# toandaominh1997/EfficientDet.Pytorch

Measured on NVIDIA H100. Metric: EfficientDet-D0 512x512 images/sec (fwd+bwd), higher is better.
Workload: dtype f32

## Files before the change

### efficientdet.pytorch_b200/csrc/conv_planes.cu

```cuda
#include "tc_ptx.cuh"

#include <stdlib.h>

namespace effdet {

constexpr int kPlMaxLevels = 8;
constexpr int kPlThreads = 384;
constexpr int kPlProducerRegs = 40, kPlConsumerRegs = 232;
constexpr int kPlA = 128 * 128;
template <int BN>
struct PlCfg {
    static constexpr int kStages = BN == 128 ? 3 : 4;
    static constexpr int kB = BN * 128;
    static constexpr int kStage = 2 * kPlA + 2 * kB;
    static constexpr int kSmem = kStages * kStage + kRowsBytes + 1024 + 256 + 2 * BN * 4;
};
constexpr int kPlBarRows = 2, kPlBarTurn = 4;

struct PlLevel {
    int B, H, W;
    WgGeom g;
    int tile_begin;
    int nboxes;
    float* y;
    long long y_bstride;
    __nv_bfloat16* y_planes;
    const __nv_bfloat16* mask_planes;
    const float* residual;
    long long r_bstride;
};
struct PlArgs {
    PlLevel lv[kPlMaxLevels];
    int nlevels, total_tiles, ntn;
    int Cin, Cout, ksize, act, kblocks, opitch;
    const float* bias;
    float* colsum;
};
struct PlMaps {
    CUtensorMap x[kPlMaxLevels];
};

template <int BN, int NP>
__global__ void __launch_bounds__(kPlThreads, 1)
conv_planes_kernel(const __grid_constant__ PlMaps maps, const __grid_constant__ CUtensorMap wmap, const __grid_constant__ PlArgs P) {
    constexpr int kPlBN = BN, kPlStages = PlCfg<BN>::kStages, kPlB = PlCfg<BN>::kB, kPlStage = PlCfg<BN>::kStage;
    extern __shared__ uint8_t smem_raw[];
    uint8_t* smem = smem_raw + ((1024u - (smem_u32(smem_raw) & 1023u)) & 1023u);
    float* rows_buf = reinterpret_cast<float*>(smem + kPlStages * kPlStage);
    uint64_t* full_bar = reinterpret_cast<uint64_t*>(smem + kPlStages * kPlStage + kRowsBytes);
    uint64_t* empty_bar = full_bar + kPlStages;
    float* chan_buf = reinterpret_cast<float*>(smem + kPlStages * kPlStage + kRowsBytes + 256);

    const int warp = threadIdx.x >> 5, lane = threadIdx.x & 31;
    const int taps = P.ksize * P.ksize, pad = P.ksize / 2;
    const int KT = taps * P.kblocks;
    if (threadIdx.x == 0) {
        for (int s = 0; s < kPlStages; ++s) {
            mbar_init(&full_bar[s], 1);
            mbar_init(&empty_bar[s], 4);
        }
        fence_barrier_init();
        tma_prefetch_desc(&wmap);
    }
    __syncthreads();

    auto decode = [&](int unit, int& l, int& box0, int& n0) {
        const int mt = unit / P.ntn;
        n0 = (unit - mt * P.ntn) * kPlBN;
        l = 0;
        while (l + 1 < P.nlevels && mt >= P.lv[l + 1].tile_begin) ++l;
        box0 = (mt - P.lv[l].tile_begin) * (128 / P.lv[l].g.kstage);
    };

    if (warp >= 8) {
        setmaxnreg_dec<kPlProducerRegs>();
        if (warp == 8 && lane == 0) {
            uint32_t it = 0;
            for (int unit = blockIdx.x; unit < P.total_tiles; unit += gridDim.x) {
                int l, box0, n0;
                decode(unit, l, box0, n0);
                const PlLevel& L = P.lv[l];
                const int ks = L.g.kstage, nbox = 128 / ks;
                const int nvalid = min(nbox, L.nboxes - box0);
                for (int kt = 0; kt < KT; ++kt, ++it) {
                    const int s = it % kPlStages;
                    const uint32_t ph = (it / kPlStages) & 1;
                    const int tap = kt / P.kblocks, kb = kt - tap * P.kblocks;
                    const int dy = tap / P.ksize - pad, dx = tap % P.ksize - pad;
                    mbar_wait(&empty_bar[s], ph ^ 1);
                    uint8_t* a_hi = smem + s * kPlStage;
                    uint8_t* b_hi = a_hi + 2 * kPlA;
                    mbar_arrive_expect_tx(&full_bar[s], (uint32_t)((NP == 3 ? 2 : 1) * (nvalid * ks * 128 + kPlB)));
                    for (int q = 0; q < nvalid; ++q) {
                        int ch = box0 + q;
                        const int bx = ch % L.g.nbx;
                        ch /= L.g.nbx;
                        const int by = ch % L.g.nby;
                        const int bb = ch / L.g.nby;
                        const int x0 = bx * L.g.Wb + dx, y0 = by * L.g.Hb + dy, b0 = bb * L.g.Bb;
                        tma_load_5d(a_hi + q * ks * 128, &maps.x[l], &full_bar[s], kb * 64, x0, y0, b0, 0);
                        if (NP == 3) tma_load_5d(a_hi + kPlA + q * ks * 128, &maps.x[l], &full_bar[s], kb * 64, x0, y0, b0, 1);
                    }
                    tma_load_3d(b_hi, &wmap, &full_bar[s], kt * 64, n0, 0);
                    if (NP == 3) tma_load_3d(b_hi + kPlB, &wmap, &full_bar[s], kt * 64, n0, 1);
                }
            }
        }
    } else {
        setmaxnreg_inc<kPlConsumerRegs>();
        constexpr int NB = kPlBN / 64;
        const int g = warp >> 2;
        const int half = (warp >> 1) & 1;
        const int etid = threadIdx.x & 127;
        float* rows = rows_buf + g * 32 * kRowsPitch;
        float* chan = chan_buf + g * kPlBN;
        const int nunits = (P.total_tiles - (int)blockIdx.x + (int)gridDim.x - 1) / (int)gridDim.x;
        int chan_n0 = -1;
        for (int k = g; k < nunits; k += 2) {
            int l, box0, n0;
            decode(blockIdx.x + k * gridDim.x, l, box0, n0);
            const PlLevel& L = P.lv[l];
            if (k > 0) named_bar_sync(kPlBarTurn + g, 256);
            float d[2][NB][32];
            uint32_t it = (uint32_t)k * KT;
            for (int kt = 0; kt < KT; ++kt, ++it) {
                const int s = it % kPlStages;
                const uint32_t ph = (it / kPlStages) & 1;
                mbar_wait(&full_bar[s], ph);
                const uint32_t sa = smem_u32(smem + s * kPlStage);
                const uint32_t sb = sa + 2 * kPlA;
                wgmma_fence();
#pragma unroll
                for (int k16 = 0; k16 < 4; ++k16) {
#pragma unroll
                    for (int m = 0; m < 2; ++m)
                        wg_mma<NB, 0, NP>(d[m], sa + m * 64 * 128 + k16 * 32, sa + kPlA + m * 64 * 128 + k16 * 32, sb + k16 * 32,
                                          sb + kPlB + k16 * 32, 16, 1024, (kt | k16) != 0);
                }
                wgmma_commit();
                wgmma_wait<1>();
                if (kt > 0 && lane == 0) mbar_arrive(&empty_bar[(it - 1) % kPlStages]);
            }
            if (k + 1 < nunits) named_bar_arrive(kPlBarTurn + (g ^ 1), 256);
            wgmma_wait<0>();
            if (lane == 0) mbar_arrive(&empty_bar[(it - 1) % kPlStages]);
            if (n0 != chan_n0) {
                named_bar_sync(kPlBarRows + g, 128);
                for (int i = etid; i < kPlBN; i += 128) chan[i] = (n0 + i < P.Cout && P.bias) ? __ldg(P.bias + n0 + i) : 0.f;
                named_bar_sync(kPlBarRows + g, 128);
                chan_n0 = n0;
            }
            const long long plane = (long long)L.B * L.H * L.W * P.opitch;
            const int ncols = min(kPlBN, P.Cout - n0);
            const int nchunks = (ncols + 31) >> 5;
#pragma unroll
            for (int m = 0; m < 2; ++m) {
                const int r = m * 64 + (warp & 1) * 32 + lane;
                const int ks = L.g.kstage;
                const int q = r / ks, i = r - q * ks;
                int ch = box0 + q;
                bool row_ok = ch < L.nboxes;
                const int bx = ch % L.g.nbx;
                ch /= L.g.nbx;
                const int by = ch % L.g.nby;
                const int bb = ch / L.g.nby;
                const int wh = L.g.Wb * L.g.Hb;
                const int bi = i / wh, rem = i - bi * wh;
                const int yy = rem / L.g.Wb, xx = rem - yy * L.g.Wb;
                const int b = bb * L.g.Bb + bi, y = by * L.g.Hb + yy, x = bx * L.g.Wb + xx;
                row_ok = row_ok && b < L.B;
// ... 248 lines not shown
```

### efficientdet.pytorch_b200/csrc/conv_tc.cu

```cuda
#include "tc_ptx.cuh"

namespace effdet {

constexpr int kTcThreads = 288;
constexpr int kTcProducers = 256;
constexpr int kTileM = 128;
constexpr int kTileK = 64;
constexpr int kWgMaxChunksPerSplit = 64;

template <int BN, int STAGES>
struct FwdSmem {
    static constexpr int kA = kTileM * 128;
    static constexpr int kB = BN * 128;
    static constexpr int kStage = 2 * kA + 2 * kB;
    static constexpr int kChan = BN * 4;
    static constexpr int kBytes = STAGES * kStage + 1024  + 256  + kChan;
};

struct ConvMultiArgs {
    ConvLevel lv[kMaxLevels];
    int tile_begin[kMaxLevels + 1];
    int nlevels;
};

// ... 126 lines not shown
        for (int jb = 0; jb < NB; ++jb) {
            float acc[32];
            wg_rows<2>(d[jb], rows_buf, g, acc);
            const int cc = 2 * jb + half;
            if (cc >= nchunks || !row_ok) continue;
#pragma unroll
            for (int q = 0; q < 8; ++q) {
                const int nl = cc * 32 + q * 4;
                const int n = n0 + nl;
                if (n >= p.Cout) break;
                float4 v = make_float4(acc[q * 4], acc[q * 4 + 1], acc[q * 4 + 2], acc[q * 4 + 3]);
                v = f4add(v, *reinterpret_cast<const float4*>(chan + nl));
                if (p.act == EFFDET_ACT_RELU) {
                    v = make_float4(fmaxf(v.x, 0.f), fmaxf(v.y, 0.f), fmaxf(v.z, 0.f), fmaxf(v.w, 0.f));
                } else if (p.act == EFFDET_ACT_SIGMOID) {
                    v = make_float4(sigmoidf_(v.x), sigmoidf_(v.y), sigmoidf_(v.z), sigmoidf_(v.w));
                } else if (p.act == EFFDET_ACT_SWISH) {
                    v = make_float4(swishf_(v.x), swishf_(v.y), swishf_(v.z), swishf_(v.w));
                }
                if (p.residual) v = f4add(v, ldg4(p.residual + rbase + n));
                if (p.mask_src) {
                    const float4 mv = ldg4(p.mask_src + mbase + n);
                    v = make_float4(mv.x > 0.f ? v.x : 0.f, mv.y > 0.f ? v.y : 0.f, mv.z > 0.f ? v.z : 0.f, mv.w > 0.f ? v.w : 0.f);
                }
                st4(p.y + ybase + n, v);
            }
        }
    } else if (warp == 8) {
        if (lane == 0) {
            for (int kt = 0; kt < KT; ++kt) {
                const int s = kt % STAGES;
                const uint32_t ph = (kt / STAGES) & 1;
                mbar_wait(&empty_bar[s], ph ^ 1);
                uint8_t* b_hi = smem + s * S::kStage + 2 * S::kA;
                mbar_arrive_expect_tx(&full_bar[s], (NP == 3 ? 2 : 1) * S::kB);
                tma_load_3d(b_hi, &wmap, &full_bar[s], kt * kTileK, n0, 0);
                if (NP == 3) tma_load_3d(b_hi + S::kB, &wmap, &full_bar[s], kt * kTileK, n0, 1);
            }
        }
    }
}

template <int BC, int STAGES>
struct WgSmem {
    static constexpr int kA = kTileK * 128 * (kTileM / 64);
    static constexpr int kB = kTileK * 128 * (BC / 64);
    static constexpr int kStage = 2 * kA + 2 * kB;
    static constexpr int kBytes = STAGES * kStage + 1024 + 256;
};

template <int NGROUPS, int NP>
__device__ __forceinline__ void wg_produce(const float* __restrict__ src, const long long bstride, const int C, const int c0,
                                           const int H, const int W, const int HW, const int M, const int mbase, const int dy,
                                           const int dx, uint8_t* hi_plane, uint8_t* lo_plane, const int t) {
    constexpr int ITEMS = 64 * NGROUPS * 8 / kTcProducers;
    const int j = t & 7;
#pragma unroll 4
    for (int it = 0; it < ITEMS; ++it) {
        const int idx = it * kTcProducers + t;
        const int rg = idx >> 3;
        const int g = rg % NGROUPS, r = rg / NGROUPS;
        const int m = mbase + r;
        const int c = c0 + g * 64 + j * 8;
        float4 v0 = f4zero(), v1 = f4zero();
        if (m < M && c < C) {
            const int b = m / HW;
            const int pix = m - b * HW;
            const int oy = pix / W;
            const int iy = oy + dy, ix = pix - oy * W + dx;
            if (iy >= 0 && iy < H && ix >= 0 && ix < W) {
                const float* q = src + (long long)b * bstride + ((long long)iy * W + ix) * C + c;
                v0 = ldg4(q);
                if (c + 4 < C) v1 = ldg4(q + 4);
            }
        }
        if constexpr (NP == 3) {
            uint4 hi, lo;
            split8(v0, v1, hi, lo);
            const int off = g * (kTileK * 128) + r * 128 + ((j ^ (r & 7)) << 4);
            *reinterpret_cast<uint4*>(hi_plane + off) = hi;
            *reinterpret_cast<uint4*>(lo_plane + off) = lo;
        } else {
            const int off = g * (kTileK * 128) + r * 128 + ((j ^ (r & 7)) << 4);
            *reinterpret_cast<uint4*>(hi_plane + off) = hi8(v0, v1);
        }
    }
}

template <int NB>
__device__ __forceinline__ void wg_atomic_dw(const float (&d)[NB][32], float* dw, const int n0, const int c0, const int Cout,
                                             const int Cin, const int kk, const int tap) {
    const int w = (threadIdx.x >> 5) & 3, lane = threadIdx.x & 31;
#pragma unroll
    for (int jb = 0; jb < NB; ++jb)
#pragma unroll
        for (int i = 0; i < 32; ++i) {
            const int n = n0 + 16 * w + (lane >> 2) + 8 * ((i >> 1) & 1);
            const int c = c0 + jb * 64 + 8 * (i >> 2) + 2 * (lane & 3) + (i & 1);
            if (n < Cout && c < Cin) atomicAdd(dw + ((long long)n * Cin + c) * kk + tap, d[jb][i]);
        }
}

template <int BC, int STAGES, int NP>
__global__ void __launch_bounds__(kTcProducers, 1)
wgrad_tc_kernel(const __grid_constant__ WgradPrefix pa, const int M, const int HW, const int chunks_per_split, const int ctiles) {
    using S = WgSmem<BC, STAGES>;
    const effdet_wgrad_args& p = pa.get();
    extern __shared__ uint8_t smem_raw[];
    uint8_t* smem = smem_raw + ((1024u - (smem_u32(smem_raw) & 1023u)) & 1023u);

    const int warp = threadIdx.x >> 5;
    const int ct = blockIdx.x % ctiles, nt = blockIdx.x / ctiles;
    const int c0 = ct * BC, n0 = nt * kTileM;
    const int tap = blockIdx.y;
    const int pad = p.ksize / 2;
    const int dy = tap / p.ksize - pad, dx = tap % p.ksize - pad;
    const int nchunks = (M + kTileK - 1) / kTileK;
    const int ch_begin = blockIdx.z * chunks_per_split;
    const int ch_end = min(nchunks, ch_begin + chunks_per_split);
    const int KT = ch_end - ch_begin;
    constexpr int NB = BC / 64;
    constexpr uint32_t GROUP = kTileK * 128;
    const int t = threadIdx.x, g = warp >> 2;
    float d[NB][32];
    for (int kt = 0; kt < KT; ++kt) {
        const int s = kt % STAGES;
        wgmma_wait<STAGES - 1>();
        named_bar_sync(1, kTcProducers);
        uint8_t* a_hi = smem + s * S::kStage;
        uint8_t* b_hi = a_hi + 2 * S::kA;
        const int mbase = (ch_begin + kt) * kTileK;
        wg_produce<kTileM / 64, NP>(p.dy, p.dy_bstride, p.Cout, n0, p.H, p.W, HW, M, mbase, 0, 0, a_hi, a_hi + S::kA, t);
        wg_produce<BC / 64, NP>(p.x, p.x_bstride, p.Cin, c0, p.H, p.W, HW, M, mbase, dy, dx, b_hi, b_hi + S::kB, t);
        fence_proxy_async();
        named_bar_sync(1, kTcProducers);
        const uint32_t sa = smem_u32(a_hi) + g * GROUP, sb = smem_u32(b_hi);
        wg_mma_mn_steps<kTileK / 16, NP>(d, sa, sa + S::kA, sb, sb + S::kB, GROUP, kt != 0);
        wgmma_commit();
    }
    wgmma_wait<0>();
    wg_atomic_dw<NB>(d, p.dw, n0 + 64 * g, c0, p.Cout, p.Cin, p.ksize * p.ksize, tap);
}

struct WgMaps {
    CUtensorMap dy[kWgMaxLevels];
    CUtensorMap x[kWgMaxLevels];
};
struct WgMultiArgs {
    WgGeom g[kWgMaxLevels];
    int chunk_begin[kWgMaxLevels + 1];
    int nlevels;
    float* dw;
    int Cin, Cout, ksize;
};

template <int BC, int STAGES, int NP>
__global__ void __launch_bounds__(kTcThreads, 1)
wgrad_tc2_multi_kernel(const __grid_constant__ WgMaps maps, const __grid_constant__ WgMultiArgs a, const int chunks_per_split,
                       const int ctiles) {
    using S = WgSmem<BC, STAGES>;
    extern __shared__ uint8_t smem_raw[];
    uint8_t* smem = smem_raw + ((1024u - (smem_u32(smem_raw) & 1023u)) & 1023u);
    uint64_t* full_bar = reinterpret_cast<uint64_t*>(smem + STAGES * S::kStage);
    uint64_t* empty_bar = full_bar + STAGES;

    const int warp = threadIdx.x >> 5, lane = threadIdx.x & 31;
    const int ct = blockIdx.x % ctiles, nt = blockIdx.x / ctiles;
    const int c0 = ct * BC, n0 = nt * kTileM;
    const int tap = blockIdx.y;
    const int pad = a.ksize / 2;
    const int dy = tap / a.ksize - pad, dx = tap % a.ksize - pad;
    const int nchunks = a.chunk_begin[a.nlevels];
    const int ch_begin = blockIdx.z * chunks_per_split;
    const int ch_end = min(nchunks, ch_begin + chunks_per_split);
    const int KT = ch_end - ch_begin;

    if (threadIdx.x == 0) {
        for (int s = 0; s < STAGES; ++s) {
            mbar_init(&full_bar[s], 1);
            mbar_init(&empty_bar[s], 8);
        }
        fence_barrier_init();
    }
    __syncthreads();
    constexpr int GROUP = kTileK * 128;

    if (warp == 8) {
        if (lane == 0) {
            int l = 0;
            for (int kt = 0; kt < KT; ++kt) {
                const int s = kt % STAGES;
                const uint32_t ph = (kt / STAGES) & 1;
                const int chg = ch_begin + kt;
                while (l + 1 < a.nlevels && chg >= a.chunk_begin[l + 1]) ++l;
                const WgGeom& g = a.g[l];
                int ch = chg - a.chunk_begin[l];
                const int bx = ch % g.nbx;
                ch /= g.nbx;
                const int by = ch % g.nby;
                const int bb = ch / g.nby;
                const int x0 = bx * g.Wb, y0 = by * g.Hb, b0 = bb * g.Bb;
                const uint32_t bytes = (uint32_t)((NP == 3 ? 2 : 1) * (kTileM / 64 + BC / 64) * g.kstage * 128);
                mbar_wait(&empty_bar[s], ph ^ 1);
                mbar_arrive_expect_tx(&full_bar[s], bytes);
                uint8_t* a_hi = smem + s * S::kStage;
                uint8_t* b_hi = a_hi + 2 * S::kA;
#pragma unroll
                for (int pl = 0; pl < (NP == 3 ? 2 : 1); ++pl) {
#pragma unroll
                    for (int q = 0; q < kTileM / 64; ++q)
                        tma_load_5d(a_hi + pl * S::kA + q * GROUP, &maps.dy[l], &full_bar[s], n0 + q * 64, x0, y0, b0, pl);
#pragma unroll
                    for (int q = 0; q < BC / 64; ++q)
                        tma_load_5d(b_hi + pl * S::kB + q * GROUP, &maps.x[l], &full_bar[s], c0 + q * 64, x0 + dx, y0 + dy, b0, pl);
                }
            }
        }
    } else {
        constexpr int NB = BC / 64;
        const int wg = warp >> 2;
        float d[NB][32];
        for (int kt = 0, l = 0; kt < KT; ++l) {
            const int end = min(KT, a.chunk_begin[l + 1] - ch_begin);
            with_count<1, 2, 3, 4>(a.g[l].kstage / 16, [&](auto ksteps) {
                for (; kt < end; ++kt) {
                    const int s = kt % STAGES;
                    const uint32_t ph = (kt / STAGES) & 1;
                    mbar_wait(&full_bar[s], ph);
                    const uint32_t sa = smem_u32(smem + s * S::kStage) + wg * GROUP;
                    const uint32_t sb = smem_u32(smem + s * S::kStage) + 2 * S::kA;
                    wg_mma_mn_steps<ksteps, NP>(d, sa, sa + S::kA, sb, sb + S::kB, GROUP, kt != 0);
                    wgmma_commit();
                    wgmma_wait<1>();
                    if (kt > 0 && lane == 0) mbar_arrive(&empty_bar[(kt - 1) % STAGES]);
                }
            });
        }
        wgmma_wait<0>();
        wg_atomic_dw<NB>(d, a.dw, n0 + 64 * wg, c0, a.Cout, a.Cin, a.ksize * a.ksize, tap);
    }
}

__global__ void pack_weight_tc_kernel(const float* __restrict__ w, __nv_bfloat16* __restrict__ out, int Cout, int Cin, int taps,
                                      int kpad, int dgrad) {
    const int rows = dgrad ? Cin : Cout;
    const int kdim = dgrad ? Cout : Cin;
    const long long plane = (long long)rows * taps * kpad;
    for (long long i = (long long)blockIdx.x * blockDim.x + threadIdx.x; i < plane; i += (long long)gridDim.x * blockDim.x) {
        const int k = (int)(i % kpad);
        const long long r2 = i / kpad;
        const int tap = (int)(r2 % taps);
        const int row = (int)(r2 / taps);
        float v = 0.f;
        if (k < kdim) {
            const int n = dgrad ? k : row, c = dgrad ? row : k;
            const int st = dgrad ? (taps - 1 - tap) : tap;
            v = __ldg(w + ((long long)n * Cin + c) * taps + st);
        }
        const __nv_bfloat16 h = __float2bfloat16_rn(v);
        out[i] = h;
        out[plane + i] = __float2bfloat16_rn(v - __bfloat162float(h));
    }
}

EncodeTiledFn encode_fn() {
    static EncodeTiledFn fn = nullptr;
    static bool tried = false;
    if (!tried) {
        tried = true;
        void* ptr = nullptr;
        cudaDriverEntryPointQueryResult q;
        if (cudaGetDriverEntryPoint("cuTensorMapEncodeTiled", &ptr, cudaEnableDefault, &q) == cudaSuccess &&
            q == cudaDriverEntryPointSuccess)
            fn = reinterpret_cast<EncodeTiledFn>(ptr);
    }
    return fn;
}

int conv_tc_kpad(int k) { return (k + kTileK - 1) / kTileK * kTileK; }

int kmajor_planes_map(EncodeTiledFn enc, CUtensorMap* map, const void* base, int rows, int k, int box_rows) {
    const cuuint64_t gdim[3] = {(cuuint64_t)k, (cuuint64_t)rows, 2};
    const cuuint64_t gstr[2] = {(cuuint64_t)k * 2, (cuuint64_t)rows * k * 2};
    const cuuint32_t box[3] = {(cuuint32_t)kTileK, (cuuint32_t)box_rows, 1};
    const cuuint32_t estr[3] = {1, 1, 1};
    CUresult r = enc(map, CU_TENSOR_MAP_DATA_TYPE_BFLOAT16, 3, const_cast<void*>(base), gdim, gstr, box, estr,
                     CU_TENSOR_MAP_INTERLEAVE_NONE, CU_TENSOR_MAP_SWIZZLE_128B, CU_TENSOR_MAP_L2_PROMOTION_L2_256B,
                     CU_TENSOR_MAP_FLOAT_OOB_FILL_NONE);
    if (r != CUDA_SUCCESS) return fail(EFFDET_ERR_LAUNCH, "tensor map of bf16 planes [2][%d][%d] failed (%d)", rows, k, (int)r);
    return EFFDET_OK;
}

int conv_tc_launch(const effdet_conv_args* levels, int nlevels, cudaStream_t st) {
    EncodeTiledFn enc = encode_fn();
    if (!enc) return fail(EFFDET_ERR_UNSUPPORTED, "conv2d(tc): cuTensorMapEncodeTiled unavailable");
    const effdet_conv_args* a = &levels[0];
    const int taps = a->ksize * a->ksize;
    const int kpad = conv_tc_kpad(a->Cin);
    const int kblocks = kpad / kTileK;
    const int BN = a->Cout <= 64 ? 64 : 128;
    CUtensorMap map;
    int s = kmajor_planes_map(enc, &map, a->w_tc, a->Cout, taps * kpad, BN);
    if (s) return s;
    ConvMultiArgs ma;
    memset(&ma, 0, sizeof(ma));
    ma.nlevels = nlevels;
    int tiles = 0;
    for (int l = 0; l < nlevels; ++l) {
        ma.lv[l].set(levels[l]);
        ma.tile_begin[l] = tiles;
        tiles += cdiv((long long)levels[l].B * levels[l].H * levels[l].W, kTileM);
    }
    for (int l = nlevels; l <= kMaxLevels; ++l) ma.tile_begin[l] = tiles;
    dim3 grid(tiles, cdiv(a->Cout, BN));
    if (a->tc_single) {
        if (BN == 64)
            return launch_smem("conv_tc_kernel", conv_tc_kernel<64, 4, 1>, grid, kTcThreads, FwdSmem<64, 4>::kBytes, st, map, ma, kblocks);
        return launch_smem("conv_tc_kernel", conv_tc_kernel<128, 3, 1>, grid, kTcThreads, FwdSmem<128, 3>::kBytes, st, map, ma, kblocks);
    }
    if (BN == 64) return launch_smem("conv_tc_kernel", conv_tc_kernel<64, 4, 3>, grid, kTcThreads, FwdSmem<64, 4>::kBytes, st, map, ma, kblocks);
    return launch_smem("conv_tc_kernel", conv_tc_kernel<128, 3, 3>, grid, kTcThreads, FwdSmem<128, 3>::kBytes, st, map, ma, kblocks);
}

bool wg_geometry(int B, int H, int W, WgGeom* g) {
    const int Wb = W <= 64 ? W : 64;
    if (W % Wb) return false;
    int Hb = 1;
    for (int h = 1; h <= H && Wb * h <= 64; ++h)
        if (H % h == 0) Hb = h;
    int Bb = 64 / (Wb * Hb);
    if (Bb < 1) Bb = 1;
    if (Bb > B) Bb = B;
    const int ks = Wb * Hb * Bb;
    if (ks < 16 || ks % 16) return false;
    g->Wb = Wb; g->Hb = Hb; g->Bb = Bb;
    g->nbx = W / Wb; g->nby = H / Hb; g->nbb = (B + Bb - 1) / Bb;
    g->kstage = ks;
    return true;
}

int planes_map(EncodeTiledFn enc, CUtensorMap* map, void* base, int B, int H, int W, int C, int pitch, const WgGeom& g) {
    const cuuint64_t gdim[5] = {(cuuint64_t)C, (cuuint64_t)W, (cuuint64_t)H, (cuuint64_t)B, 2};
    const cuuint64_t gstr[4] = {(cuuint64_t)pitch * 2, (cuuint64_t)W * pitch * 2, (cuuint64_t)H * W * pitch * 2,
                                (cuuint64_t)B * H * W * pitch * 2};
    const cuuint32_t box[5] = {64, (cuuint32_t)g.Wb, (cuuint32_t)g.Hb, (cuuint32_t)g.Bb, 1};
    const cuuint32_t estr[5] = {1, 1, 1, 1, 1};
    CUresult r = enc(map, CU_TENSOR_MAP_DATA_TYPE_BFLOAT16, 5, base, gdim, gstr, box, estr, CU_TENSOR_MAP_INTERLEAVE_NONE,
                     CU_TENSOR_MAP_SWIZZLE_128B, CU_TENSOR_MAP_L2_PROMOTION_L2_256B, CU_TENSOR_MAP_FLOAT_OOB_FILL_NONE);
    if (r != CUDA_SUCCESS) return fail(EFFDET_ERR_LAUNCH, "wgrad(tc): cuTensorMapEncodeTiled failed (%d)", (int)r);
    return EFFDET_OK;
}

int wgrad_tc2_launch(const effdet_wgrad_args* levels, int nlevels, cudaStream_t st) {
    EncodeTiledFn enc = encode_fn();
    WgMaps maps;
    WgMultiArgs ma;
    memset(&ma, 0, sizeof(ma));
    const effdet_wgrad_args* a0 = &levels[0];
    const int cin_pad = conv_tc_kpad(a0->Cin), cout_pad = conv_tc_kpad(a0->Cout);
    int chunks = 0;
    for (int l = 0; l < nlevels; ++l) {
        const effdet_wgrad_args* a = &levels[l];
        wg_geometry(a->B, a->H, a->W, &ma.g[l]);
        ma.chunk_begin[l] = chunks;
        chunks += ma.g[l].nbx * ma.g[l].nby * ma.g[l].nbb;
    }
    for (int l = nlevels; l <= kWgMaxLevels; ++l) ma.chunk_begin[l] = chunks;
    ma.nlevels = nlevels;
    ma.dw = a0->dw;
    ma.Cin = a0->Cin; ma.Cout = a0->Cout; ma.ksize = a0->ksize;
    for (int l = 0; l < nlevels; ++l) {
        const effdet_wgrad_args* a = &levels[l];
        const int HW = a->H * a->W;
        int s = EFFDET_OK;
        if (a->x_planes) {
            if ((s = planes_map(enc, &maps.x[l], const_cast<void*>(a->x_planes), a->B, a->H, a->W, a->Cin, (a->Cin + 7) / 8 * 8, ma.g[l])))
                return s;
        } else {
            if ((s = to_planes_launch(a->x, a->x_bstride, nullptr, 0, a->ws_x, nullptr, a->B, HW, a->Cin, cin_pad, st))) return s;
            if ((s = planes_map(enc, &maps.x[l], a->ws_x, a->B, a->H, a->W, cin_pad, cin_pad, ma.g[l]))) return s;
        }
        if (a->dy_planes) {
            if ((s = planes_map(enc, &maps.dy[l], const_cast<void*>(a->dy_planes), a->B, a->H, a->W, a->Cout, (a->Cout + 7) / 8 * 8,
                                ma.g[l])))
                return s;
        } else {
            if ((s = to_planes_launch(a->dy, a->dy_bstride, nullptr, 0, a->ws_dy, a->dbias, a->B, HW, a->Cout, cout_pad, st))) return s;
            if ((s = planes_map(enc, &maps.dy[l], a->ws_dy, a->B, a->H, a->W, cout_pad, cout_pad, ma.g[l]))) return s;
        }
    }
    for (int l = nlevels; l < kWgMaxLevels; ++l) { maps.dy[l] = maps.dy[0]; maps.x[l] = maps.x[0]; }
    const int taps = a0->ksize * a0->ksize;
    const int BC = a0->Cin > 64 ? 256 : 64;
    const int ctiles = cdiv(a0->Cin, BC), ntiles = cdiv(a0->Cout, kTileM);
    int splits = (num_sms() * 2) / (ctiles * ntiles * taps);
    if (splits < 1) splits = 1;
    if (splits > cdiv(chunks, 4)) splits = cdiv(chunks, 4);
    if (splits < cdiv(chunks, kWgMaxChunksPerSplit)) splits = cdiv(chunks, kWgMaxChunksPerSplit);
    int cps = cdiv(chunks, splits);
    splits = cdiv(chunks, cps);
    dim3 grid(ctiles * ntiles, taps, splits);
    if (a0->tc_single) {
        if (BC == 256)
            return launch_smem("wgrad_tc2_multi_kernel", wgrad_tc2_multi_kernel<256, 2, 1>, grid, kTcThreads, WgSmem<256, 2>::kBytes,
                               st, maps, ma, cps, ctiles);
        return launch_smem("wgrad_tc2_multi_kernel", wgrad_tc2_multi_kernel<64, 4, 1>, grid, kTcThreads, WgSmem<64, 4>::kBytes, st,
                           maps, ma, cps, ctiles);
    }
    if (BC == 256)
        return launch_smem("wgrad_tc2_multi_kernel", wgrad_tc2_multi_kernel<256, 2, 3>, grid, kTcThreads, WgSmem<256, 2>::kBytes, st,
                           maps, ma, cps, ctiles);
    return launch_smem("wgrad_tc2_multi_kernel", wgrad_tc2_multi_kernel<64, 4, 3>, grid, kTcThreads, WgSmem<64, 4>::kBytes, st, maps,
                       ma, cps, ctiles);
}

int wgrad_tc_launch(const effdet_wgrad_args* a, cudaStream_t st) {
    const int M = a->B * a->H * a->W, HW = a->H * a->W;
    const int taps = a->ksize * a->ksize;
    const int BC = a->Cin > 64 ? 256 : 64;
    const int ctiles = cdiv(a->Cin, BC), ntiles = cdiv(a->Cout, kTileM);
    const int nchunks = cdiv(M, kTileK);
    int splits = cdiv(num_sms() * 2, ctiles * ntiles * taps);
    if (splits < 1) splits = 1;
    if (splits > cdiv(nchunks, 8)) splits = cdiv(nchunks, 8);
    if (splits < cdiv(nchunks, kWgMaxChunksPerSplit)) splits = cdiv(nchunks, kWgMaxChunksPerSplit);
    int cps = cdiv(nchunks, splits);
    splits = cdiv(nchunks, cps);
    dim3 grid(ctiles * ntiles, taps, splits);
    WgradPrefix pa;
    pa.set(*a);
    if (a->tc_single) {
        if (BC == 256)
            return launch_smem("wgrad_tc_kernel", wgrad_tc_kernel<256, 2, 1>, grid, kTcProducers, WgSmem<256, 2>::kBytes, st, pa, M, HW,
                               cps, ctiles);
        return launch_smem("wgrad_tc_kernel", wgrad_tc_kernel<64, 4, 1>, grid, kTcProducers, WgSmem<64, 4>::kBytes, st, pa, M, HW, cps,
                           ctiles);
    }
    if (BC == 256)
        return launch_smem("wgrad_tc_kernel", wgrad_tc_kernel<256, 2, 3>, grid, kTcProducers, WgSmem<256, 2>::kBytes, st, pa, M, HW, cps,
                           ctiles);
    return launch_smem("wgrad_tc_kernel", wgrad_tc_kernel<64, 4, 3>, grid, kTcProducers, WgSmem<64, 4>::kBytes, st, pa, M, HW, cps, ctiles);
}

}

using namespace effdet;

extern "C" int effdet_conv_tc_kpad(int channels) { return conv_tc_kpad(channels); }
extern "C" int effdet_wgrad_tc_geometry_ok(int B, int H, int W) {
    WgGeom g;
    return wg_geometry(B, H, W, &g) ? 1 : 0;
}

extern "C" int effdet_pack_conv_weight_tc(const float* w_oihw, void* w_fwd, void* w_dgrad, int Cout, int Cin, int ksize,
                                          int device, effdet_stream_t stream) {
    EFFDET_REQUIRE(w_oihw && w_fwd && Cout > 0 && Cin > 0 && (ksize == 1 || ksize == 3), "pack_conv_weight_tc: bad arguments");
    EFFDET_DEVICE(device);
    const int taps = ksize * ksize;
    cudaStream_t st = (cudaStream_t)stream;
    {
        const int kpad = conv_tc_kpad(Cin);
        const long long plane = (long long)Cout * taps * kpad;
        int blocks = cdiv(plane, 256);
        if (blocks > num_sms() * 8) blocks = num_sms() * 8;
        pack_weight_tc_kernel<<<blocks, 256, 0, st>>>(w_oihw, (__nv_bfloat16*)w_fwd, Cout, Cin, taps, kpad, 0);
        int s = launch_status("pack_weight_tc_kernel");
        if (s) return s;
    }
    if (w_dgrad) {
        const int kpad = conv_tc_kpad(Cout);
        const long long plane = (long long)Cin * taps * kpad;
        int blocks = cdiv(plane, 256);
        if (blocks > num_sms() * 8) blocks = num_sms() * 8;
        pack_weight_tc_kernel<<<blocks, 256, 0, st>>>(w_oihw, (__nv_bfloat16*)w_dgrad, Cout, Cin, taps, kpad, 1);
        return launch_status("pack_weight_tc_kernel");
    }
    return EFFDET_OK;
}
```

### efficientdet.pytorch_b200/csrc/tc_ptx.cuh

```cuda
#pragma once
#include "common.cuh"

#include <cuda.h>
#include <cuda_bf16.h>
#include <stddef.h>
#include <type_traits>

namespace effdet {

__device__ __forceinline__ uint32_t smem_u32(const void* p) { return (uint32_t)__cvta_generic_to_shared(p); }

__device__ __forceinline__ void mbar_init(uint64_t* bar, uint32_t count) {
    asm volatile("mbarrier.init.shared::cta.b64 [%0], %1;" ::"r"(smem_u32(bar)), "r"(count));
}
__device__ __forceinline__ void mbar_arrive(uint64_t* bar) {
    asm volatile("mbarrier.arrive.shared::cta.b64 _, [%0];" ::"r"(smem_u32(bar)) : "memory");
}
__device__ __forceinline__ void mbar_arrive_expect_tx(uint64_t* bar, uint32_t bytes) {
    asm volatile("mbarrier.arrive.expect_tx.shared::cta.b64 _, [%0], %1;" ::"r"(smem_u32(bar)), "r"(bytes) : "memory");
}
__device__ __forceinline__ void mbar_wait(uint64_t* bar, uint32_t parity) {
    const uint32_t a = smem_u32(bar);
    uint32_t done;
    do {
        asm volatile(
            "{\n\t.reg .pred p;\n\t"
            "mbarrier.try_wait.parity.shared::cta.b64 p, [%1], %2;\n\t"
            "selp.u32 %0, 1, 0, p;\n\t}"
            : "=r"(done)
            : "r"(a), "r"(parity)
            : "memory");
    } while (!done);
}
__device__ __forceinline__ void fence_barrier_init() { asm volatile("fence.mbarrier_init.release.cluster;" ::: "memory"); }
__device__ __forceinline__ void fence_proxy_async() { asm volatile("fence.proxy.async.shared::cta;" ::: "memory"); }
__device__ __forceinline__ void tma_load_3d(void* dst, const CUtensorMap* map, uint64_t* bar, int c0, int c1, int c2) {
    asm volatile(
        "cp.async.bulk.tensor.3d.shared::cluster.global.tile.mbarrier::complete_tx::bytes [%0], [%1, {%3, %4, %5}], [%2];"
        ::"r"(smem_u32(dst)), "l"(reinterpret_cast<uint64_t>(map)), "r"(smem_u32(bar)), "r"(c0), "r"(c1), "r"(c2)
        : "memory");
}

__device__ __forceinline__ void tma_load_5d(void* dst, const CUtensorMap* map, uint64_t* bar, int c0, int c1, int c2, int c3, int c4) {
    asm volatile(
        "cp.async.bulk.tensor.5d.shared::cluster.global.tile.mbarrier::complete_tx::bytes [%0], [%1, {%3, %4, %5, %6, %7}], [%2];"
        ::"r"(smem_u32(dst)), "l"(reinterpret_cast<uint64_t>(map)), "r"(smem_u32(bar)), "r"(c0), "r"(c1), "r"(c2), "r"(c3), "r"(c4)
        : "memory");
}


__device__ __forceinline__ uint64_t gmma_desc(uint32_t smem_addr, uint32_t lbo_bytes, uint32_t sbo_bytes) {
    return (uint64_t)((smem_addr >> 4) & 0x3FFF) | ((uint64_t)((lbo_bytes >> 4) & 0x3FFF) << 16) |
           ((uint64_t)((sbo_bytes >> 4) & 0x3FFF) << 32) | (1ull << 62);
}
__device__ __forceinline__ void wgmma_fence() { asm volatile("wgmma.fence.sync.aligned;" ::: "memory"); }
__device__ __forceinline__ void wgmma_commit() { asm volatile("wgmma.commit_group.sync.aligned;" ::: "memory"); }
template <int N>
__device__ __forceinline__ void wgmma_wait() {
    asm volatile("wgmma.wait_group.sync.aligned %0;" ::"n"(N) : "memory");
}
#define EFFDET_WG_D8(a, o) "+f"(a[o]), "+f"(a[o + 1]), "+f"(a[o + 2]), "+f"(a[o + 3]), "+f"(a[o + 4]), "+f"(a[o + 5]), \
                           "+f"(a[o + 6]), "+f"(a[o + 7])
#define EFFDET_WG_D32(a) EFFDET_WG_D8(a, 0), EFFDET_WG_D8(a, 8), EFFDET_WG_D8(a, 16), EFFDET_WG_D8(a, 24)
template <int MN>
__device__ __forceinline__ void wgmma_bf16(float (&d)[1][32], uint64_t desc_a, uint64_t desc_b, uint32_t accumulate) {
    asm volatile(
        "{\n\t.reg .pred p;\n\t"
        "setp.ne.b32 p, %34, 0;\n\t"
        "wgmma.mma_async.sync.aligned.m64n64k16.f32.bf16.bf16 {"
        "%0, %1, %2, %3, %4, %5, %6, %7, %8, %9, %10, %11, %12, %13, %14, %15, "
        "%16, %17, %18, %19, %20, %21, %22, %23, %24, %25, %26, %27, %28, %29, %30, %31"
        "}, %32, %33, p, 1, 1, %35, %35;\n\t}"
        : EFFDET_WG_D32(d[0])
        : "l"(desc_a), "l"(desc_b), "r"(accumulate), "n"(MN)
        : "memory");
}
template <int MN>
__device__ __forceinline__ void wgmma_bf16(float (&d)[2][32], uint64_t desc_a, uint64_t desc_b, uint32_t accumulate) {
    asm volatile(
        "{\n\t.reg .pred p;\n\t"
        "setp.ne.b32 p, %66, 0;\n\t"
        "wgmma.mma_async.sync.aligned.m64n128k16.f32.bf16.bf16 {"
        "%0, %1, %2, %3, %4, %5, %6, %7, %8, %9, %10, %11, %12, %13, %14, %15, "
        "%16, %17, %18, %19, %20, %21, %22, %23, %24, %25, %26, %27, %28, %29, %30, %31, "
        "%32, %33, %34, %35, %36, %37, %38, %39, %40, %41, %42, %43, %44, %45, %46, %47, "
        "%48, %49, %50, %51, %52, %53, %54, %55, %56, %57, %58, %59, %60, %61, %62, %63"
        "}, %64, %65, p, 1, 1, %67, %67;\n\t}"
        : EFFDET_WG_D32(d[0]), EFFDET_WG_D32(d[1])
        : "l"(desc_a), "l"(desc_b), "r"(accumulate), "n"(MN)
        : "memory");
}
template <int MN>
__device__ __forceinline__ void wgmma_bf16(float (&d)[4][32], uint64_t desc_a, uint64_t desc_b, uint32_t accumulate) {
    asm volatile(
        "{\n\t.reg .pred p;\n\t"
        "setp.ne.b32 p, %130, 0;\n\t"
        "wgmma.mma_async.sync.aligned.m64n256k16.f32.bf16.bf16 {"
        "%0, %1, %2, %3, %4, %5, %6, %7, %8, %9, %10, %11, %12, %13, %14, %15, "
        "%16, %17, %18, %19, %20, %21, %22, %23, %24, %25, %26, %27, %28, %29, %30, %31, "
        "%32, %33, %34, %35, %36, %37, %38, %39, %40, %41, %42, %43, %44, %45, %46, %47, "
        "%48, %49, %50, %51, %52, %53, %54, %55, %56, %57, %58, %59, %60, %61, %62, %63, "
        "%64, %65, %66, %67, %68, %69, %70, %71, %72, %73, %74, %75, %76, %77, %78, %79, "
        "%80, %81, %82, %83, %84, %85, %86, %87, %88, %89, %90, %91, %92, %93, %94, %95, "
        "%96, %97, %98, %99, %100, %101, %102, %103, %104, %105, %106, %107, %108, %109, %110, %111, "
        "%112, %113, %114, %115, %116, %117, %118, %119, %120, %121, %122, %123, %124, %125, %126, %127"
        "}, %128, %129, p, 1, 1, %131, %131;\n\t}"
        : EFFDET_WG_D32(d[0]), EFFDET_WG_D32(d[1]), EFFDET_WG_D32(d[2]), EFFDET_WG_D32(d[3])
        : "l"(desc_a), "l"(desc_b), "r"(accumulate), "n"(MN)
        : "memory");
}
#undef EFFDET_WG_D32
#undef EFFDET_WG_D8
template <int NB, int MN, int P>
__device__ __forceinline__ void wg_mma(float (&d)[NB][32], uint32_t a_hi, uint32_t a_lo, uint32_t b_hi, uint32_t b_lo,
                                       uint32_t lbo, uint32_t sbo, uint32_t accumulate) {
    static_assert(P == 1 || P == 3, "one or three bf16 products per multiply-add");
    if constexpr (P == 3) {
        const uint64_t dah = gmma_desc(a_hi, lbo, sbo), dal = gmma_desc(a_lo, lbo, sbo);
        const uint64_t dbh = gmma_desc(b_hi, lbo, sbo), dbl = gmma_desc(b_lo, lbo, sbo);
        wgmma_bf16<MN>(d, dal, dbh, accumulate);
        wgmma_bf16<MN>(d, dah, dbl, 1);
        wgmma_bf16<MN>(d, dah, dbh, 1);
    } else {
        wgmma_bf16<MN>(d, gmma_desc(a_hi, lbo, sbo), gmma_desc(b_hi, lbo, sbo), accumulate);
    }
}
template <int KS, int P, int NB>
__device__ __forceinline__ void wg_mma_mn_steps(float (&d)[NB][32], uint32_t a_hi, uint32_t a_lo, uint32_t b_hi, uint32_t b_lo,
                                                uint32_t group, uint32_t accumulate) {
    wgmma_fence();
#pragma unroll
    for (int k = 0; k < KS; ++k) {
        const uint32_t ko = k * 2 * 1024;
        wg_mma<NB, 1, P>(d, a_hi + ko, a_lo + ko, b_hi + ko, b_lo + ko, group, 1024, accumulate | k);
    }
}
template <int... KS, class F>
__device__ __forceinline__ void with_count(const int n, F&& f) {
    (void)((n == KS && (f(std::integral_constant<int, KS>()), true)) || ...);
}

__device__ __forceinline__ void named_bar_sync(int id, int nthreads) {
    asm volatile("bar.sync %0, %1;" ::"r"(id), "r"(nthreads) : "memory");
}
template <int N>
__device__ __forceinline__ void setmaxnreg_dec() {
    asm volatile("setmaxnreg.dec.sync.aligned.u32 %0;" ::"n"(N));
}
template <int N>
__device__ __forceinline__ void setmaxnreg_inc() {
    asm volatile("setmaxnreg.inc.sync.aligned.u32 %0;" ::"n"(N));
}
__device__ __forceinline__ void named_bar_arrive(int id, int nthreads) {
    asm volatile("bar.arrive %0, %1;" ::"r"(id), "r"(nthreads) : "memory");
}

constexpr int kRowsPitch = 68;
constexpr int kRowsBytes = 64 * kRowsPitch * 4;
template <int NWG>
__device__ __forceinline__ void wg_rows(const float (&d)[32], float* buf, const int g, float (&out)[32]) {
    const int w = (threadIdx.x >> 5) & 3, lane = threadIdx.x & 31;
#pragma unroll 1
    for (int turn = 0; turn < NWG; ++turn) {
        named_bar_sync(1, NWG * 128);
        if (turn != g) continue;
#pragma unroll
        for (int i = 0; i < 32; i += 2) {
            const int row = 16 * w + (lane >> 2) + 8 * ((i >> 1) & 1), col = 8 * (i >> 2) + 2 * (lane & 3);
            *reinterpret_cast<float2*>(buf + row * kRowsPitch + col) = make_float2(d[i], d[i + 1]);
        }
        named_bar_sync(2 + g, 128);
        const float* src = buf + ((w & 1) * 32 + lane) * kRowsPitch + (w >> 1) * 32;
#pragma unroll
        for (int q = 0; q < 8; ++q) {
            const float4 v = *reinterpret_cast<const float4*>(src + 4 * q);
            out[4 * q] = v.x; out[4 * q + 1] = v.y; out[4 * q + 2] = v.z; out[4 * q + 3] = v.w;
        }
    }
}
__device__ __forceinline__ void wg_rows_own(const float (&d)[32], float* buf, const int bar, float (&out)[32]) {
    const int w = (threadIdx.x >> 5) & 3, lane = threadIdx.x & 31;
#pragma unroll 1
    for (int h = 0; h < 2; ++h) {
        named_bar_sync(bar, 128);
        if ((w >> 1) == h) {
#pragma unroll
            for (int i = 0; i < 32; i += 2) {
                const int row = 16 * (w & 1) + (lane >> 2) + 8 * ((i >> 1) & 1), col = 8 * (i >> 2) + 2 * (lane & 3);
                *reinterpret_cast<float2*>(buf + row * kRowsPitch + col) = make_float2(d[i], d[i + 1]);
            }
        }
        named_bar_sync(bar, 128);
        if ((w & 1) == h) {
            const float* src = buf + lane * kRowsPitch + (w >> 1) * 32;
#pragma unroll
            for (int q = 0; q < 8; ++q) {
                const float4 v = *reinterpret_cast<const float4*>(src + 4 * q);
                out[4 * q] = v.x; out[4 * q + 1] = v.y; out[4 * q + 2] = v.z; out[4 * q + 3] = v.w;
            }
        }
    }
}

__device__ __forceinline__ void split8(const float4 a, const float4 b, uint4& hi, uint4& lo) {
    const float f[8] = {a.x, a.y, a.z, a.w, b.x, b.y, b.z, b.w};
    uint32_t h[4], l[4];
#pragma unroll
    for (int i = 0; i < 4; ++i) {
        const __nv_bfloat162 hh = __floats2bfloat162_rn(f[2 * i], f[2 * i + 1]);
        const float r0 = f[2 * i] - __low2float(hh), r1 = f[2 * i + 1] - __high2float(hh);
        const __nv_bfloat162 ll = __floats2bfloat162_rn(r0, r1);
        h[i] = *reinterpret_cast<const uint32_t*>(&hh);
        l[i] = *reinterpret_cast<const uint32_t*>(&ll);
    }
    hi = make_uint4(h[0], h[1], h[2], h[3]);
    lo = make_uint4(l[0], l[1], l[2], l[3]);
}
__device__ __forceinline__ uint4 hi8(const float4 a, const float4 b) {
    const __nv_bfloat162 h0 = __floats2bfloat162_rn(a.x, a.y), h1 = __floats2bfloat162_rn(a.z, a.w);
    const __nv_bfloat162 h2 = __floats2bfloat162_rn(b.x, b.y), h3 = __floats2bfloat162_rn(b.z, b.w);
    return make_uint4(*reinterpret_cast<const uint32_t*>(&h0), *reinterpret_cast<const uint32_t*>(&h1),
                      *reinterpret_cast<const uint32_t*>(&h2), *reinterpret_cast<const uint32_t*>(&h3));
}


__device__ __forceinline__ void tma_load_2d(void* dst, const CUtensorMap* map, uint64_t* bar, int c0, int c1) {
    asm volatile(
        "cp.async.bulk.tensor.2d.shared::cluster.global.tile.mbarrier::complete_tx::bytes [%0], [%1, {%3, %4}], [%2];"
        ::"r"(smem_u32(dst)), "l"(reinterpret_cast<uint64_t>(map)), "r"(smem_u32(bar)), "r"(c0), "r"(c1)
        : "memory");
}
__device__ __forceinline__ void tma_prefetch_desc(const CUtensorMap* map) {
    asm volatile("prefetch.tensormap [%0];" ::"l"(reinterpret_cast<uint64_t>(map)) : "memory");
}
typedef CUresult (*EncodeTiledFn)(CUtensorMap*, CUtensorMapDataType, cuuint32_t, void*, const cuuint64_t*, const cuuint64_t*,
                                  const cuuint32_t*, const cuuint32_t*, CUtensorMapInterleave, CUtensorMapSwizzle,
                                  CUtensorMapL2promotion, CUtensorMapFloatOOBfill);
EncodeTiledFn encode_fn();
int conv_tc_kpad(int k);
int kmajor_planes_map(EncodeTiledFn enc, CUtensorMap* map, const void* base, int rows, int k, int box_rows);
int to_planes_launch(const float* x, long long x_bstride, const float* prob, long long p_bstride, void* out, float* colsum,
                     int B, int HW, int C, int pitch, cudaStream_t st);

template <class... P, class... A>
int launch_smem(const char* name, void (*kernel)(P...), dim3 grid, int threads, size_t smem, cudaStream_t st, const A&... args) {
    const cudaError_t e = cudaFuncSetAttribute(kernel, cudaFuncAttributeMaxDynamicSharedMemorySize, (int)smem);
    if (e != cudaSuccess) return fail(EFFDET_ERR_LAUNCH, "%s: smem opt-in: %s", name, cudaGetErrorString(e));
    kernel<<<grid, threads, smem, st>>>(args...);
    return launch_status(name);
}

template <class T, size_t N>
struct alignas(8) ArgsPrefix {
    unsigned char raw[N];
    __host__ __device__ const T& get() const { return *reinterpret_cast<const T*>(raw); }
    void set(const T& a) { memcpy(raw, &a, N); }
};
using ConvLevel = ArgsPrefix<effdet_conv_args, offsetof(effdet_conv_args, tc_single)>;
using WgradPrefix = ArgsPrefix<effdet_wgrad_args, offsetof(effdet_wgrad_args, tc_single)>;

constexpr int kMaxLevels = 8;
constexpr int kWgMaxLevels = 8;

struct WgGeom {
    int Wb, Hb, Bb;
    int nbx, nby, nbb;
    int kstage;
};
bool wg_geometry(int B, int H, int W, WgGeom* g);
int planes_map(EncodeTiledFn enc, CUtensorMap* map, void* base, int B, int H, int W, int C, int pitch, const WgGeom& g);

}
```

Measured before the change: 534.4.

## Make wgrad kernel persistent with ping-pong consumer warpgroups and register rebalancing

```diff
diff --git a/efficientdet.pytorch_b200/csrc/conv_planes.cu b/efficientdet.pytorch_b200/csrc/conv_planes.cu
--- a/efficientdet.pytorch_b200/csrc/conv_planes.cu
+++ b/efficientdet.pytorch_b200/csrc/conv_planes.cu
@@ -5,8 +5,6 @@
 namespace effdet {
 
 constexpr int kPlMaxLevels = 8;
-constexpr int kPlThreads = 384;
-constexpr int kPlProducerRegs = 40, kPlConsumerRegs = 232;
 constexpr int kPlA = 128 * 128;
 template <int BN>
 struct PlCfg {
@@ -15,7 +13,7 @@
     static constexpr int kStage = 2 * kPlA + 2 * kB;
     static constexpr int kSmem = kStages * kStage + kRowsBytes + 1024 + 256 + 2 * BN * 4;
 };
-constexpr int kPlBarRows = 2, kPlBarTurn = 4;
+constexpr int kPlBarRows = 2;
 
 struct PlLevel {
     int B, H, W;
diff --git a/efficientdet.pytorch_b200/csrc/conv_tc.cu b/efficientdet.pytorch_b200/csrc/conv_tc.cu
--- a/efficientdet.pytorch_b200/csrc/conv_tc.cu
+++ b/efficientdet.pytorch_b200/csrc/conv_tc.cu
@@ -302,12 +302,15 @@
     int nlevels;
     float* dw;
     int Cin, Cout, ksize;
+    int chunks_per_split, ctiles, ntiles, units;
 };
-
-template <int BC, int STAGES, int NP>
-__global__ void __launch_bounds__(kTcThreads, 1)
-wgrad_tc2_multi_kernel(const __grid_constant__ WgMaps maps, const __grid_constant__ WgMultiArgs a, const int chunks_per_split,
-                       const int ctiles) {
+template <int BC>
+constexpr int kWgStages = BC == 128 ? 3 : 4;
+
+template <int BC, int MS, int NP>
+__global__ void __launch_bounds__(kPlThreads, 1)
+wgrad_tc2_multi_kernel(const __grid_constant__ WgMaps maps, const __grid_constant__ WgMultiArgs a) {
+    constexpr int STAGES = kWgStages<BC>;
     using S = WgSmem<BC, STAGES>;
     extern __shared__ uint8_t smem_raw[];
     uint8_t* smem = smem_raw + ((1024u - (smem_u32(smem_raw) & 1023u)) & 1023u);
@@ -315,79 +318,109 @@
     uint64_t* empty_bar = full_bar + STAGES;
 
     const int warp = threadIdx.x >> 5, lane = threadIdx.x & 31;
-    const int ct = blockIdx.x % ctiles, nt = blockIdx.x / ctiles;
-    const int c0 = ct * BC, n0 = nt * kTileM;
-    const int tap = blockIdx.y;
-    const int pad = a.ksize / 2;
-    const int dy = tap / a.ksize - pad, dx = tap % a.ksize - pad;
+    const int taps = a.ksize * a.ksize, pad = a.ksize / 2;
     const int nchunks = a.chunk_begin[a.nlevels];
-    const int ch_begin = blockIdx.z * chunks_per_split;
-    const int ch_end = min(nchunks, ch_begin + chunks_per_split);
-    const int KT = ch_end - ch_begin;
-
     if (threadIdx.x == 0) {
         for (int s = 0; s < STAGES; ++s) {
             mbar_init(&full_bar[s], 1);
-            mbar_init(&empty_bar[s], 8);
+            mbar_init(&empty_bar[s], 4);
         }
         fence_barrier_init();
     }
     __syncthreads();
     constexpr int GROUP = kTileK * 128;
 
-    if (warp == 8) {
-        if (lane == 0) {
-            int l = 0;
-            for (int kt = 0; kt < KT; ++kt) {
-                const int s = kt % STAGES;
-                const uint32_t ph = (kt / STAGES) & 1;
-                const int chg = ch_begin + kt;
-                while (l + 1 < a.nlevels && chg >= a.chunk_begin[l + 1]) ++l;
-                const WgGeom& g = a.g[l];
-                int ch = chg - a.chunk_begin[l];
-                const int bx = ch % g.nbx;
-                ch /= g.nbx;
-                const int by = ch % g.nby;
-                const int bb = ch / g.nby;
-                const int x0 = bx * g.Wb, y0 = by * g.Hb, b0 = bb * g.Bb;
-                const uint32_t bytes = (uint32_t)((NP == 3 ? 2 : 1) * (kTileM / 64 + BC / 64) * g.kstage * 128);
-                mbar_wait(&empty_bar[s], ph ^ 1);
-                mbar_arrive_expect_tx(&full_bar[s], bytes);
-                uint8_t* a_hi = smem + s * S::kStage;
-                uint8_t* b_hi = a_hi + 2 * S::kA;
-#pragma unroll
-                for (int pl = 0; pl < (NP == 3 ? 2 : 1); ++pl) {
-#pragma unroll
-                    for (int q = 0; q < kTileM / 64; ++q)
-                        tma_load_5d(a_hi + pl * S::kA + q * GROUP, &maps.dy[l], &full_bar[s], n0 + q * 64, x0, y0, b0, pl);
-#pragma unroll
-                    for (int q = 0; q < BC / 64; ++q)
-                        tma_load_5d(b_hi + pl * S::kB + q * GROUP, &maps.x[l], &full_bar[s], c0 + q * 64, x0 + dx, y0 + dy, b0, pl);
+    auto decode = [&](int unit, int& ch0, int& n, int& tap, int& n0, int& c0) {
+        c0 = unit % a.ctiles * BC;
+        unit /= a.ctiles;
+        n0 = unit % a.ntiles * kTileM;
+        unit /= a.ntiles;
+        tap = unit % taps;
+        ch0 = unit / taps * a.chunks_per_split;
+        n = min(nchunks - ch0, a.chunks_per_split);
+    };
+
+    if (warp >= 8) {
+        setmaxnreg_dec<kPlProducerRegs>();
+        if (warp == 8 && lane == 0) {
+            uint32_t it = 0;
+            for (int unit = blockIdx.x; unit < a.units; unit += gridDim.x) {
+                int ch0, n, tap, n0, c0;
+                decode(unit, ch0, n, tap, n0, c0);
+                const int dy = tap / a.ksize - pad, dx = tap % a.ksize - pad;
+                int l = 0;
+                for (int chg = ch0; chg < ch0 + n; ++chg, ++it) {
+                    const int s = it % STAGES;
+                    const uint32_t ph = (it / STAGES) & 1;
+                    while (l + 1 < a.nlevels && chg >= a.chunk_begin[l + 1]) ++l;
+                    const WgGeom& g = a.g[l];
+                    int ch = chg - a.chunk_begin[l];
+                    const int bx = ch % g.nbx;
+                    ch /= g.nbx;
+                    const int by = ch % g.nby;
+                    const int bb = ch / g.nby;
+                    const int x0 = bx * g.Wb, y0 = by * g.Hb, b0 = bb * g.Bb;
+                    const uint32_t bytes = (uint32_t)((NP == 3 ? 2 : 1) * (MS + BC / 64) * g.kstage * 128);
+                    mbar_wait(&empty_bar[s], ph ^ 1);
+                    mbar_arrive_expect_tx(&full_bar[s], bytes);
+                    uint8_t* a_hi = smem + s * S::kStage;
+                    uint8_t* b_hi = a_hi + 2 * S::kA;
+#pragma unroll
+                    for (int pl = 0; pl < (NP == 3 ? 2 : 1); ++pl) {
+#pragma unroll
+                        for (int q = 0; q < MS; ++q)
+                            tma_load_5d(a_hi + pl * S::kA + q * GROUP, &maps.dy[l], &full_bar[s], n0 + q * 64, x0, y0, b0, pl);
+#pragma unroll
+                        for (int q = 0; q < BC / 64; ++q)
+                            tma_load_5d(b_hi + pl * S::kB + q * GROUP, &maps.x[l], &full_bar[s], c0 + q * 64, x0 + dx, y0 + dy, b0, pl);
+                    }
                 }
             }
         }
     } else {
+        setmaxnreg_inc<kPlConsumerRegs>();
         constexpr int NB = BC / 64;
-        const int wg = warp >> 2;
-        float d[NB][32];
-        for (int kt = 0, l = 0; kt < KT; ++l) {
-            const int end = min(KT, a.chunk_begin[l + 1] - ch_begin);
-            with_count<1, 2, 3, 4>(a.g[l].kstage / 16, [&](auto ksteps) {
-                for (; kt < end; ++kt) {
-                    const int s = kt % STAGES;
-                    const uint32_t ph = (kt / STAGES) & 1;
-                    mbar_wait(&full_bar[s], ph);
-                    const uint32_t sa = smem_u32(smem + s * S::kStage) + wg * GROUP;
-                    const uint32_t sb = smem_u32(smem + s * S::kStage) + 2 * S::kA;
-                    wg_mma_mn_steps<ksteps, NP>(d, sa, sa + S::kA, sb, sb + S::kB, GROUP, kt != 0);
-                    wgmma_commit();
-                    wgmma_wait<1>();
-                    if (kt > 0 && lane == 0) mbar_arrive(&empty_bar[(kt - 1) % STAGES]);
-                }
-            });
-        }
-        wgmma_wait<0>();
-        wg_atomic_dw<NB>(d, a.dw, n0 + 64 * wg, c0, a.Cout, a.Cin, a.ksize * a.ksize, tap);
+        const int g = warp >> 2;
+        const int nunits = (a.units - (int)blockIdx.x + (int)gridDim.x - 1) / (int)gridDim.x;
+        uint32_t it = 0;
+        for (int k = 0; k < nunits; ++k) {
+            int ch0, n, tap, n0, c0;
+            decode(blockIdx.x + k * gridDim.x, ch0, n, tap, n0, c0);
+            if ((k & 1) != g) {
+                it += n;
+                continue;
+            }
+            if (k > 0) named_bar_sync(kPlBarTurn + g, 256);
+            float d[MS][NB][32];
+            for (int kt = 0, l = 0; kt < n; ++l) {
+                const int end = min(n, a.chunk_begin[l + 1] - ch0);
+                with_count<1, 2, 3, 4>(a.g[l].kstage / 16, [&](auto ksteps) {
+                    for (; kt < end; ++kt, ++it) {
+                        const int s = it % STAGES;
+                        const uint32_t ph = (it / STAGES) & 1;
+                        mbar_wait(&full_bar[s], ph);
+                        const uint32_t sa = smem_u32(smem + s * S::kStage), sb = sa + 2 * S::kA;
+                        wgmma_fence();
+#pragma unroll
+                        for (int k16 = 0; k16 < decltype(ksteps)::value; ++k16) {
+                            const uint32_t ko = k16 * 2 * 1024;
+#pragma unroll
+                            for (int m = 0; m < MS; ++m)
+                                wg_mma<NB, 1, NP>(d[m], sa + m * GROUP + ko, sa + S::kA + m * GROUP + ko, sb + ko, sb + S::kB + ko,
+                                                  GROUP, 1024, (kt | k16) != 0);
+                        }
+                        wgmma_commit();
+                        wgmma_wait<1>();
+                        if (kt > 0 && lane == 0) mbar_arrive(&empty_bar[(it - 1) % STAGES]);
+                    }
+                });
+            }
+            if (k + 1 < nunits) named_bar_arrive(kPlBarTurn + (g ^ 1), 256);
+            wgmma_wait<0>();
+            if (lane == 0) mbar_arrive(&empty_bar[(it - 1) % STAGES]);
+#pragma unroll
+            for (int m = 0; m < MS; ++m) wg_atomic_dw<NB>(d[m], a.dw, n0 + 64 * m, c0, a.Cout, a.Cin, taps, tap);
+        }
     }
 }
 
@@ -541,27 +574,35 @@
     }
     for (int l = nlevels; l < kWgMaxLevels; ++l) { maps.dy[l] = maps.dy[0]; maps.x[l] = maps.x[0]; }
     const int taps = a0->ksize * a0->ksize;
-    const int BC = a0->Cin > 64 ? 256 : 64;
-    const int ctiles = cdiv(a0->Cin, BC), ntiles = cdiv(a0->Cout, kTileM);
-    int splits = (num_sms() * 2) / (ctiles * ntiles * taps);
+    const int ntiles = cdiv(a0->Cout, kTileM);
+    const int plan_ctiles = cdiv(a0->Cin, a0->Cin > 64 ? 256 : 64);
+    int splits = (num_sms() * 2) / (plan_ctiles * ntiles * taps);
     if (splits < 1) splits = 1;
     if (splits > cdiv(chunks, 4)) splits = cdiv(chunks, 4);
     if (splits < cdiv(chunks, kWgMaxChunksPerSplit)) splits = cdiv(chunks, kWgMaxChunksPerSplit);
     int cps = cdiv(chunks, splits);
     splits = cdiv(chunks, cps);
-    dim3 grid(ctiles * ntiles, taps, splits);
+    const int BC = a0->Cin > 64 ? 128 : 64;
+    ma.chunks_per_split = cps;
+    ma.ctiles = cdiv(a0->Cin, BC);
+    ma.ntiles = ntiles;
+    ma.units = splits * taps * ntiles * ma.ctiles;
+    const int grid = ma.units < num_sms() ? ma.units : num_sms();
+    const bool m1 = a0->Cout <= 64;
+    const size_t smem = BC == 128 ? WgSmem<128, kWgStages<128>>::kBytes : WgSmem<64, kWgStages<64>>::kBytes;
+    const char* name = "wgrad_tc2_multi_kernel";
     if (a0->tc_single) {
-        if (BC == 256)
-            return launch_smem("wgrad_tc2_multi_kernel", wgrad_tc2_multi_kernel<256, 2, 1>, grid, kTcThreads, WgSmem<256, 2>::kBytes,
-                               st, maps, ma, cps, ctiles);
-        return launch_smem("wgrad_tc2_multi_kernel", wgrad_tc2_multi_kernel<64, 4, 1>, grid, kTcThreads, WgSmem<64, 4>::kBytes, st,
-                           maps, ma, cps, ctiles);
-    }
-    if (BC == 256)
-        return launch_smem("wgrad_tc2_multi_kernel", wgrad_tc2_multi_kernel<256, 2, 3>, grid, kTcThreads, WgSmem<256, 2>::kBytes, st,
-                           maps, ma, cps, ctiles);
-    return launch_smem("wgrad_tc2_multi_kernel", wgrad_tc2_multi_kernel<64, 4, 3>, grid, kTcThreads, WgSmem<64, 4>::kBytes, st, maps,
-                       ma, cps, ctiles);
+        if (BC == 128)
+            return m1 ? launch_smem(name, wgrad_tc2_multi_kernel<128, 1, 1>, grid, kPlThreads, smem, st, maps, ma)
+                      : launch_smem(name, wgrad_tc2_multi_kernel<128, 2, 1>, grid, kPlThreads, smem, st, maps, ma);
+        return m1 ? launch_smem(name, wgrad_tc2_multi_kernel<64, 1, 1>, grid, kPlThreads, smem, st, maps, ma)
+                  : launch_smem(name, wgrad_tc2_multi_kernel<64, 2, 1>, grid, kPlThreads, smem, st, maps, ma);
+    }
+    if (BC == 128)
+        return m1 ? launch_smem(name, wgrad_tc2_multi_kernel<128, 1, 3>, grid, kPlThreads, smem, st, maps, ma)
+                  : launch_smem(name, wgrad_tc2_multi_kernel<128, 2, 3>, grid, kPlThreads, smem, st, maps, ma);
+    return m1 ? launch_smem(name, wgrad_tc2_multi_kernel<64, 1, 3>, grid, kPlThreads, smem, st, maps, ma)
+              : launch_smem(name, wgrad_tc2_multi_kernel<64, 2, 3>, grid, kPlThreads, smem, st, maps, ma);
 }
 
 int wgrad_tc_launch(const effdet_wgrad_args* a, cudaStream_t st) {
diff --git a/efficientdet.pytorch_b200/csrc/tc_ptx.cuh b/efficientdet.pytorch_b200/csrc/tc_ptx.cuh
--- a/efficientdet.pytorch_b200/csrc/tc_ptx.cuh
+++ b/efficientdet.pytorch_b200/csrc/tc_ptx.cuh
@@ -155,6 +155,10 @@
     asm volatile("bar.arrive %0, %1;" ::"r"(id), "r"(nthreads) : "memory");
 }
 
+constexpr int kPlThreads = 384;
+constexpr int kPlProducerRegs = 40, kPlConsumerRegs = 232;
+constexpr int kPlBarTurn = 4;
+
 constexpr int kRowsPitch = 68;
 constexpr int kRowsBytes = 64 * kRowsPitch * 4;
 template <int NWG>
```

Result: faster. 550.2, median of 6 (+3.0%).
